# EBI-Metagenomics/deciphon

Hardware: AMD Instinct MI355X
Metric: GCUPS (Viterbi DP cell updates/sec) (higher is better)
Workload: dtype f32

## Files before the change

deciphon_amd/csrc/dcp_types.h:

```cpp
#pragma once
#include <stdint.h>

#define DCP_TABLE_SIZE 1364
#define DCP_NUM_TRANS 8
#define DCP_NUM_XTRANS 13
#define DCP_XT_STRIDE 16
#define DCP_REF_LANES 8
#define DCP_MODEL_MAX 16384

enum { DCP_BM, DCP_MM, DCP_MI, DCP_MD, DCP_IM, DCP_II, DCP_DM, DCP_DD };
enum { DCP_RR, DCP_SN, DCP_NN, DCP_SB, DCP_NB, DCP_EB, DCP_JB, DCP_EJ, DCP_JJ, DCP_EC, DCP_CC, DCP_ET, DCP_CT };

struct DcpCodeRow
{
  uint32_t c[8];
};

#define DCP_SP_STRIDE 8
#define DCP_ROW_HDR 4
#define DCP_MAX_STRIPS 8

struct DcpProfileDev
{
  int32_t K;
  int32_t Kp;
  int32_t Q;
  int32_t W;
  int64_t rows_off;
  int64_t trans_off;
  int64_t pad0, pad1;
};

struct DcpProblem
{
  int32_t profile;
  int32_t L;
  int64_t code_row;
  int32_t xt_row;
  int32_t out;
  int64_t trellis;
};

struct DcpPack
{
  int32_t profile;
  int32_t Lmax;
  int32_t L[16];
  int32_t xt_row[16];
  int32_t out[16];
  uint32_t code_row[16];
};

#ifdef __HIPCC__
#define DCP_HDI __host__ __device__ inline
// ... 25 lines not shown
```

deciphon_amd/csrc/engine.cpp:

```cpp
#include "../../include/deciphon_hip.h"
#include "dcp_db.h"
#include "dcp_errors.h"
#include "dcp_types.h"
#include "host_logic.h"
#include "viterbi_kernels.h"

#include <algorithm>
#include <atomic>
#include <deque>
#include <math.h>
#include <stdio.h>
#include <stdlib.h>
#include <string.h>
#include <string>
#include <thread>
#include <vector>

namespace
{

template <class T> struct DevBuf
{
  T *p = nullptr;
  size_t cap = 0;
// ... 90 lines not shown
    }
    auto const t0 = std::chrono::steady_clock::now();
    unsigned char *p = nullptr;
    if (hipMalloc((void **)&p, want) != hipSuccess)
    {
      (void)hipGetLastError();
      return nullptr;
    }
    double const ms = std::chrono::duration<double, std::milli>(std::chrono::steady_clock::now() - t0).count();
    alloc_ms += ms;
    if (getenv("DECIPHON_HIP_TIMING")) fprintf(stderr, "TableArena: chunk %zu, %.2f GB in %.1f ms\n", chunks.size(), (double)want / 1e9, ms);
    chunks.push_back(Chunk{p, want, bytes});
    held += want;
    placed += bytes;
    return p;
  }
};

struct HostProfile
{
  int K, Kp, Q, W, cls;
  int pack = -1;
  bool narrow = false;
  int64_t pool_off;
  std::string accession;
};

struct PathResult
{
  int K = 0, L = 0;
  float score = 0;
  size_t trellis_off = 0;
  bool has_trellis = false;
  bool trellis_on_host = false;
  uint32_t const *steps = nullptr;
  int32_t nsteps = 0;
  std::vector<uint32_t> owned;
};

}

struct dcp_hip
{
  int device = 0;
  hipStream_t stream = nullptr;
  hipStream_t qstream[DCP_NUM_CLASSES] = {nullptr};
// ... 657 lines not shown
  for (int b = 0; b < 3; ++b)
  {
    if (x->bank[b].done_ev) (void)hipEventDestroy(x->bank[b].done_ev);
    if (x->bank[b].up_ev) (void)hipEventDestroy(x->bank[b].up_ev);
  }
  for (int c = 0; c < DCP_NUM_PACK_SHAPES; ++c)
  {
    if (x->pstream[c]) (void)hipStreamDestroy(x->pstream[c]);
    if (x->pjoin_ev[c]) (void)hipEventDestroy(x->pjoin_ev[c]);
  }
  for (int c = 0; c < DCP_NUM_CLASSES; ++c)
  {
    if (x->nstream[c]) (void)hipStreamDestroy(x->nstream[c]);
    if (x->njoin_ev[c]) (void)hipEventDestroy(x->njoin_ev[c]);
  }
  if (x->fork_ev) (void)hipEventDestroy(x->fork_ev);
  if (x->stream) (void)hipStreamDestroy(x->stream);
  delete x;
}

char const *dcp_hip_strerror(struct dcp_hip const *x) { return x ? x->err.c_str() : "no engine"; }


static size_t profile_floats(int Kp)
{
  size_t const floats = (size_t)DCP_TABLE_SIZE * ((size_t)Kp + DCP_ROW_HDR) + (size_t)DCP_NUM_TRANS * (size_t)Kp;
  return (floats + 3) & ~(size_t)3;
}

static int describe(dcp_hip *x, int K, char const *accession, HostProfile &hp)
{
  if (K < 1 || K > DCP_MODEL_MAX) return fail(x, DCP_ELARGECORESIZE, "core size out of range");
  int const cls = dcp_class_of(K);
  if (cls < 0) return fail(x, DCP_ELARGECORESIZE, "core size beyond DCP_MAX_CORE_SIZE (16383: state ids keep 14 bits for k + 1)");
  hp.K = K;
  hp.cls = cls;
  dcp_class_shape(cls, &hp.Q, &hp.W);
  hp.Kp = 64 * hp.Q * hp.W;
  if (cls == DCP_STRIP_CLASS) hp.Kp *= (K + hp.Kp - 1) / hp.Kp;
  hp.pool_off = 0;
  hp.accession = accession ? accession : "";
  hp.narrow = K <= dcp_class_narrow_limit(cls);
  hp.pack = dcp_pack_shape_of(K);
  if (hp.pack >= 0)
  {
    int pq = 0, ps = 0;
    dcp_pack_shape(hp.pack, &pq, &ps);
    if (hp.W != 1 || ps * pq > hp.Kp) hp.pack = -1;
  }
  return 0;
}

static int ensure_pool(dcp_hip *x, size_t floats)
{
  if (floats <= x->d_pool.cap) return 0;
  HIP_TRY(x, hipStreamSynchronize(x->stream), DCP_EFUNCUSE);
  DevBuf<float> bigger;
  HIP_TRY(x, bigger.reserve(std::max(floats, x->d_pool.cap + x->d_pool.cap / 2)), DCP_ENOMEM);
  if (x->pool_used)
    HIP_TRY(x, hipMemcpy(bigger.p, x->d_pool.p, x->pool_used * sizeof(float), hipMemcpyDeviceToDevice), DCP_EFUNCUSE);
  x->d_pool.release();
  x->d_pool.p = bigger.p;
  x->d_pool.cap = bigger.cap;
  bigger.p = nullptr;
  bigger.cap = 0;
// ... 12 lines not shown
  x->profiles.push_back(hp);
  ++x->gen;
  return 0;
}

static bool delete_costs_ok(float const *trans, int K, int Kp)
{
  for (int k = 0; k < K; ++k)
    if (!(trans[(size_t)DCP_MD * Kp + k] >= 0.0f) || !(trans[(size_t)DCP_DD * Kp + k] >= 0.0f)) return false;
  return true;
}

int dcp_hip_add_profile(struct dcp_hip *x, int K, float const *trans, float const *match, float const *null_cost,
                        float const *bg_cost, int *index)
{
  if (!x || !trans || !match || !null_cost || !bg_cost) return DCP_EFUNCUSE;
  if (outstanding_batches(x)) return fail(x, DCP_EFUNCUSE, "cost batches are outstanding (dcp_hip_cost_hits_begin): end them first");
  HIP_TRY(x, hipSetDevice(x->device), DCP_EFUNCUSE);
  HostProfile hp;
  int rc = describe(x, K, nullptr, hp);
  if (rc) return rc;
  int const Kp = hp.Kp;
  size_t const stride = (size_t)Kp + DCP_ROW_HDR;
  std::vector<float> buf(profile_floats(Kp), INFINITY);
  float *r = buf.data();
  float *t = r + (size_t)DCP_TABLE_SIZE * stride;
  for (int id = 0; id < DCP_NUM_TRANS; ++id) memcpy(t + (size_t)id * Kp, trans + (size_t)id * K, sizeof(float) * K);
  if (!delete_costs_ok(t, K, Kp)) return fail(x, DCP_EFUNCUSE, "negative (or NaN) delete cost: costs are -log-probabilities");
  for (int c = 0; c < DCP_TABLE_SIZE; ++c)
  {
    float *hdr = r + (size_t)c * stride;
    hdr[0] = null_cost[c];
    hdr[1] = bg_cost[c];
    hdr[2] = hdr[3] = 0.0f;
    memcpy(hdr + DCP_ROW_HDR, match + (size_t)c * K, sizeof(float) * K);
  }
  return push_profile(x, hp, buf, index);
}

int dcp_hip_add_protein(struct dcp_hip *x, int K, float const *node_trans, float const *node_emission,
                        float const *BMk, float const *null_lprob, float const *bg_lprob, int *index)
{
  if (!x || !node_trans || !node_emission || !BMk || !null_lprob || !bg_lprob) return DCP_EFUNCUSE;
  if (outstanding_batches(x)) return fail(x, DCP_EFUNCUSE, "cost batches are outstanding (dcp_hip_cost_hits_begin): end them first");
  HIP_TRY(x, hipSetDevice(x->device), DCP_EFUNCUSE);
  HostProfile hp;
  int rc = describe(x, K, nullptr, hp);
  if (rc) return rc;
  std::vector<float> buf(profile_floats(hp.Kp), INFINITY);
  float *r = buf.data();
  float *t = r + (size_t)DCP_TABLE_SIZE * ((size_t)hp.Kp + DCP_ROW_HDR);
  dcp_setup_profile(K, hp.Kp, node_trans, node_emission, BMk, null_lprob, bg_lprob, t, r);
  if (!delete_costs_ok(t, K, hp.Kp)) return fail(x, DCP_EFDATA, "positive (or NaN) delete log-probability in the protein");
  return push_profile(x, hp, buf, index);
}

int dcp_hip_load_dcp(struct dcp_hip *x, char const *path, int first, int count)
{
  if (!x || !path) return DCP_EFUNCUSE;
  if (outstanding_batches(x)) return fail(x, DCP_EFUNCUSE, "cost batches are outstanding (dcp_hip_cost_hits_begin): end them first");
  HIP_TRY(x, hipSetDevice(x->device), DCP_EFUNCUSE);
  DcpDbReader db;
  int rc = db.open(path);
  if (rc) return fail(x, rc, "cannot open database");
  int const N = db.num_proteins();
  if (first < 0 || first > N) return fail(x, DCP_EINVALPART, "first protein out of range");
  int const last = count < 0 ? N : std::min(N, first + count);
  int const n = last - first;
  if (n <= 0)
  {
    ++x->gen;
    return 0;
  }

  std::vector<HostProfile> hps((size_t)n);
  std::vector<size_t> off((size_t)n + 1, 0);
  for (int i = 0; i < n; ++i)
  {
    int K = 0;
    std::string acc;
    if ((rc = db.read_protein_head(first + i, K, acc))) return fail(x, rc, "cannot read protein");
    if ((rc = describe(x, K, acc.c_str(), hps[(size_t)i]))) return rc;
    off[(size_t)i + 1] = off[(size_t)i] + profile_floats(hps[(size_t)i].Kp);
  }
  if ((rc = ensure_pool(x, x->pool_used + off[(size_t)n]))) return rc;

  size_t chunk_floats = std::max<size_t>((size_t)64 << 20, profile_floats(DCP_MAX_CORE_SIZE));
  if (char const *e = getenv("DECIPHON_HIP_STAGE_MB"))
  {
    size_t largest = 0;
    for (int i = 0; i < n; ++i) largest = std::max(largest, off[(size_t)i + 1] - off[(size_t)i]);
    chunk_floats = std::max<size_t>(((size_t)std::max(atol(e), 1L) << 20) / sizeof(float), largest);
  }
  int chunks = 0;
  float *stage[2] = {nullptr, nullptr};
  hipEvent_t done[2] = {nullptr, nullptr};
  bool busy[2] = {false, false};
  auto cleanup = [&]() {
    (void)hipStreamSynchronize(x->stream);
    for (int b = 0; b < 2; ++b)
    {
      if (stage[b]) (void)hipHostFree(stage[b]);
      if (done[b]) (void)hipEventDestroy(done[b]);
    }
  };
  for (int b = 0; b < 2; ++b)
  {
    if (hipHostMalloc((void **)&stage[b], std::min(chunk_floats, off[(size_t)n]) * sizeof(float), hipHostMallocDefault) !=
            hipSuccess ||
        hipEventCreateWithFlags(&done[b], hipEventDisableTiming) != hipSuccess)
// ... 14 lines not shown
    }
    float *buf = stage[b];
    std::atomic<int> next_protein{i0}, bad{0};
    auto work = [&]() {
      DcpProtein p;
      for (int i = next_protein.fetch_add(1); i < i1; i = next_protein.fetch_add(1))
      {
        int r = db.read_protein(first + i, p);
        if (r || p.core_size != hps[(size_t)i].K)
        {
          int expected = 0;
          bad.compare_exchange_strong(expected, r ? r : DCP_EFDATA);
          continue;
        }
        float *rows = buf + (off[(size_t)i] - off[(size_t)i0]);
        float *trans = rows + (size_t)DCP_TABLE_SIZE * ((size_t)hps[(size_t)i].Kp + DCP_ROW_HDR);
        dcp_setup_profile(p.core_size, hps[(size_t)i].Kp, p.trans.data(), p.emission.data(), p.BMk.data(),
                          p.null_emission.data(), p.bg_emission.data(), trans, rows);
        if (!delete_costs_ok(trans, p.core_size, hps[(size_t)i].Kp))
        {
          int expected = 0;
          bad.compare_exchange_strong(expected, DCP_EFDATA);
        }
      }
    };
    {
      unsigned nthreads = std::min<unsigned>({std::max(1u, std::thread::hardware_concurrency()), 16u, (unsigned)(i1 - i0)});
      std::vector<std::thread> pool;
      for (unsigned t = 1; t < nthreads; ++t) pool.emplace_back(work);
      work();
      for (std::thread &t : pool) t.join();
    }
    if (bad)
    {
      cleanup();
      return fail(x, bad, "cannot read protein");
    }
    size_t const floats = off[(size_t)i1] - off[(size_t)i0];
    if (hipMemcpyAsync(x->d_pool.p + x->pool_used + off[(size_t)i0], buf, floats * sizeof(float), hipMemcpyHostToDevice,
                       x->stream) != hipSuccess ||
        hipEventRecord(done[b], x->stream) != hipSuccess)
    {
      cleanup();
      return fail(x, DCP_EFUNCUSE, "staging copy failed");
    }
    busy[b] = true;
// ... 29 lines not shown
{
  if (!x || i < 0 || i >= (int)x->profiles.size()) return nullptr;
  return x->profiles[(size_t)i].accession.c_str();
}

int dcp_hip_commit_profiles(struct dcp_hip *x)
{
  if (!x) return DCP_EFUNCUSE;
  if (outstanding_batches(x)) return fail(x, DCP_EFUNCUSE, "cost batches are outstanding (dcp_hip_cost_hits_begin): end them first");
  HIP_TRY(x, hipSetDevice(x->device), DCP_EFUNCUSE);
  ++x->gen;
  if (x->committed == x->profiles.size()) return 0;
  HIP_TRY(x, hipStreamSynchronize(x->stream), DCP_EFUNCUSE);
  std::vector<DcpProfileDev> dev(x->profiles.size());
  for (size_t i = 0; i < dev.size(); ++i)
  {
    HostProfile const &hp = x->profiles[i];
    dev[i].K = hp.K;
    dev[i].Kp = hp.Kp;
    dev[i].Q = hp.Q;
    dev[i].W = hp.W;
    dev[i].rows_off = hp.pool_off;
    dev[i].trans_off = dev[i].rows_off + (int64_t)DCP_TABLE_SIZE * (hp.Kp + DCP_ROW_HDR);
    dev[i].pad0 = dev[i].pad1 = 0;
  }
  HIP_TRY(x, x->d_profiles.reserve(dev.size()), DCP_ENOMEM);
  HIP_TRY(x, hipMemcpyAsync(x->d_profiles.p, dev.data(), dev.size() * sizeof(DcpProfileDev), hipMemcpyHostToDevice,
                            x->stream),
          DCP_EFUNCUSE);
  HIP_TRY(x, hipStreamSynchronize(x->stream), DCP_EFUNCUSE);
  x->committed = x->profiles.size();
  return 0;
}

void dcp_hip_clear_profiles(struct dcp_hip *x)
{
  if (!x) return;
  if (outstanding_batches(x))
  {
    (void)refuse_outstanding(x);
    return;
  }
  ++x->gen;
  x->pool_used = 0;
  x->profiles.clear();
  x->committed = 0;
}
// ... 857 lines not shown
```

deciphon_amd/csrc/host_capi.cpp:

```cpp
#include "../../include/deciphon_host.h"
#include "dcp_db.h"
#include "dcp_errors.h"
#include "host_logic.h"

#include <string.h>
#include <string>
#include <vector>

struct dcp_db
{
  DcpDbReader reader;
};

extern "C" {

int dcp_db_open(char const *path, struct dcp_db **out)
{
  if (!path || !out) return DCP_EFUNCUSE;
  dcp_db *x = new dcp_db;
  int rc = x->reader.open(path);
  if (rc)
  {
    delete x;
    *out = nullptr;
// ... 55 lines not shown
int dcp_db_read_nuclt_dist(struct dcp_db const *x, int i, float *nucltp, float *codonm, int *gencode)
{
  if (!x) return DCP_EFUNCUSE;
  DcpDecoder d;
  int rc = x->reader.read_decoder(i, d);
  if (rc) return rc;
  if (nucltp) memcpy(nucltp, d.nucltp.data(), d.nucltp.size() * sizeof(float));
  if (codonm) memcpy(codonm, d.codonm.data(), d.codonm.size() * sizeof(float));
  if (gencode) *gencode = d.gencode;
  return 0;
}

int dcp_decode_quasi_codon(float epsilon, float const *nucltp4, float const *codonm125, uint8_t const *nt, int n,
                           uint8_t codon[3])
{
  if (!nucltp4 || !codonm125 || !nt || !codon) return DCP_EFUNCUSE;
  for (int i = 0; i < n && i < 5; ++i)
    if (nt[i] > 3) return DCP_ESEQABC;
  return dcp_decode_codon(epsilon, nucltp4, codonm125, nt, n, codon) ? 0 : DCP_EDECODON;
}

char dcp_gencode_amino_of(int gencode_id, uint8_t const codon[3]) { return dcp_gencode_amino(gencode_id, codon); }

int dcp_partition_bounds_of(int n, int32_t const *core_sizes, int nparts, int balanced, int32_t *first)
{
  if (n < 0 || !first || (balanced && n > 0 && !core_sizes)) return DCP_EFUNCUSE;
  if (nparts < 1) return DCP_EZEROPART;
  dcp_partition_bounds(n, core_sizes, nparts, balanced != 0, first);
  return 0;
}

int dcp_db_read_protein(struct dcp_db const *x, int i, float *node_trans, float *node_emission, float *BMk,
                        float *null_lprob, float *bg_lprob, char *accession, char *consensus)
{
  if (!x) return DCP_EFUNCUSE;
  DcpProtein p;
  int rc = x->reader.read_protein(i, p);
  if (rc) return rc;
  if (node_trans) memcpy(node_trans, p.trans.data(), p.trans.size() * sizeof(float));
  if (node_emission) memcpy(node_emission, p.emission.data(), p.emission.size() * sizeof(float));
  if (BMk) memcpy(BMk, p.BMk.data(), p.BMk.size() * sizeof(float));
  if (null_lprob) memcpy(null_lprob, p.null_emission.data(), p.null_emission.size() * sizeof(float));
  if (bg_lprob) memcpy(bg_lprob, p.bg_emission.data(), p.bg_emission.size() * sizeof(float));
  if (accession)
  {
    strncpy(accession, p.accession.c_str(), 31);
// ... 64 lines not shown
```

deciphon_amd/csrc/host_logic.cpp:

```cpp
#include "host_logic.h"
#include "../../include/deciphon_host.h"
#include "dcp_errors.h"

#include <algorithm>
#include <initializer_list>
#include <limits.h>
#include <math.h>
#include <stdio.h>
#include <string.h>
#include <utility>

void dcp_xtrans(int seq_size, bool multi_hits, bool hmmer3_compat, float xt[DCP_NUM_XTRANS])
{
  float const L = (float)seq_size;
  float q = 0.0f;
  float log_q = -INFINITY;
  if (multi_hits)
  {
    q = 0.5f;
    log_q = (float)log(0.5);
  }
  float const denom = L + 2 + q / (1 - q);
  float const two_q = 2 + q / (1 - q);
  float const Lp1 = L + 1;
// ... 31 lines not shown
  for (int k = 0; k + 1 < K; ++k)
  {
    float const *t = node_trans + 7 * (size_t)k;
    trans[DCP_MM * Kp + k + 1] = -t[0];
    trans[DCP_MI * Kp + k] = -t[1];
    trans[DCP_MD * Kp + k + 1] = -t[2];
    trans[DCP_IM * Kp + k + 1] = -t[3];
    trans[DCP_II * Kp + k] = -t[4];
    trans[DCP_DM * Kp + k + 1] = -t[5];
    trans[DCP_DD * Kp + k + 1] = -t[6];
  }
  trans[DCP_MI * Kp + K - 1] = INFINITY;
  trans[DCP_II * Kp + K - 1] = INFINITY;
  size_t const stride = (size_t)Kp + DCP_ROW_HDR;
  for (int c = 0; c < DCP_TABLE_SIZE; ++c)
  {
    float *hdr = rows + (size_t)c * stride;
    hdr[0] = -null_lprob[c];
    hdr[1] = -bg_lprob[c];
    hdr[2] = hdr[3] = 0.0f;
    float *row = hdr + DCP_ROW_HDR;
    for (int k = 0; k < K; ++k) row[k] = -node_emission[(size_t)k * DCP_TABLE_SIZE + c];
    for (int k = K; k < Kp; ++k) row[k] = INFINITY;
  }
}

int dcp_encode_sequence(char const *data, int64_t n, uint8_t *out)
{
  enum { A, C, G, T, U, NSYM };
  int64_t count[NSYM] = {0};
  for (int64_t i = 0; i < n; ++i)
  {
    switch (data[i] & ~0x20)
    {
    case 'A': count[A]++; break;
    case 'C': count[C]++; break;
    case 'G': count[G]++; break;
    case 'T': count[T]++; break;
    case 'U': count[U]++; break;
    default: break;
    }
  }
  if (count[T] > 0 && count[U] > 0) return DCP_ENUCLTSEQTU;

  auto pick = [&](std::initializer_list<int> set) {
    int best = *set.begin();
// ... 482 lines not shown
```

deciphon_amd/csrc/host_logic.h:

```cpp
#pragma once
#include "dcp_types.h"
#include <stdint.h>
#include <string>
#include <vector>

void dcp_xtrans(int seq_size, bool multi_hits, bool hmmer3_compat, float xt[DCP_NUM_XTRANS]);

void dcp_setup_profile(int K, int Kp, float const *node_trans, float const *node_emission, float const *BMk,
                       float const *null_lprob, float const *bg_lprob, float *trans, float *rows);

int dcp_encode_sequence(char const *data, int64_t n, uint8_t *out);

int dcp_unzip(int K, int L, uint32_t const *xnodes, uint16_t const *nodes, std::vector<int32_t> &state_ids,
              std::vector<int32_t> &seqsizes);

void dcp_state_name(int state_id, char name[8]);
bool dcp_state_is_mute(int state_id);

struct DcpHit
{
  int hit_start, hit_stop;
  int begin_step, end_step;
  int last_hit_pos;
};
bool dcp_find_hit(std::vector<int32_t> const &state_ids, std::vector<int32_t> const &seqsizes, DcpHit &hit);
bool dcp_find_hit_packed(uint32_t const *steps, int n, DcpHit &hit);

struct DcpWindow
{
  int core_size, seq_size;
  int start = -1, stop = 0, idx = -1, last_hit_pos = -1;
  DcpWindow(int seq_size_, int core_size_) : core_size(core_size_), seq_size(seq_size_) {}
// ... 21 lines not shown
```

deciphon_amd/csrc/lane_ops_gpu.h:

```cpp
#pragma once
#include <hip/hip_runtime.h>
#include <stdint.h>
#include <type_traits>

#include "dcp_types.h"

#define DCP_FN __device__ __forceinline__
#define DCP_WAVE 64

typedef float lf;
typedef uint32_t lu;
typedef bool lm;

DCP_FN lf lf_splat(float x) { return x; }
DCP_FN lu lu_splat(uint32_t x) { return x; }
DCP_FN lf lmin(lf a, lf b) { return __builtin_fminf(a, b); }
DCP_FN lf lmin3(lf a, lf b, lf c) { return __builtin_fminf(__builtin_fminf(a, b), c); }
DCP_FN lm llt(lf a, lf b) { return a < b; }
DCP_FN lm llt_u(lu a, lu b) { return a < b; }
DCP_FN lm leq(lf a, lf b) { return a == b; }
DCP_FN lm lequ(lu a, lu b) { return a == b; }
DCP_FN lm land(lm a, lm b) { return a && b; }
DCP_FN lm lor(lm a, lm b) { return a || b; }
DCP_FN lm lnot(lm a) { return !a; }
// ... 499 lines not shown
  dcp_u32x2 const b = __builtin_amdgcn_raw_buffer_load_b64(r.rsrc, voff + 16u, soff, 0);
  out[0] = __uint_as_float(a.x); out[1] = __uint_as_float(a.y); out[2] = __uint_as_float(a.z);
  out[3] = __uint_as_float(a.w); out[4] = __uint_as_float(b.x); out[5] = __uint_as_float(b.y);
}
template <> DCP_FN void load_row_q<8>(RowSrc const &r, lu voff, uint32_t soff, lf (&out)[8])
{
  dcp_u32x4 const a = __builtin_amdgcn_raw_buffer_load_b128(r.rsrc, voff, soff, 0);
  dcp_u32x4 const b = __builtin_amdgcn_raw_buffer_load_b128(r.rsrc, voff + 16u, soff, 0);
  out[0] = __uint_as_float(a.x); out[1] = __uint_as_float(a.y); out[2] = __uint_as_float(a.z);
  out[3] = __uint_as_float(a.w); out[4] = __uint_as_float(b.x); out[5] = __uint_as_float(b.y);
  out[6] = __uint_as_float(b.z); out[7] = __uint_as_float(b.w);
}

template <> DCP_FN void load_row_q<10>(RowSrc const &r, lu voff, uint32_t soff, lf (&out)[10])
{
  dcp_u32x4 const a = __builtin_amdgcn_raw_buffer_load_b128(r.rsrc, voff, soff, 0);
  dcp_u32x4 const b = __builtin_amdgcn_raw_buffer_load_b128(r.rsrc, voff + 16u, soff, 0);
  dcp_u32x2 const c = __builtin_amdgcn_raw_buffer_load_b64(r.rsrc, voff + 32u, soff, 0);
  out[0] = __uint_as_float(a.x); out[1] = __uint_as_float(a.y); out[2] = __uint_as_float(a.z);
  out[3] = __uint_as_float(a.w); out[4] = __uint_as_float(b.x); out[5] = __uint_as_float(b.y);
  out[6] = __uint_as_float(b.z); out[7] = __uint_as_float(b.w); out[8] = __uint_as_float(c.x);
  out[9] = __uint_as_float(c.y);
}
template <int Q> DCP_FN void store_q(float *__restrict__ row, lu lane, lf const (&v)[Q])
{
  typedef float dcp_f32x2 __attribute__((ext_vector_type(2)));
  typedef float dcp_f32x4 __attribute__((ext_vector_type(4)));
  float *p = row + (size_t)lane * Q;
  if constexpr (Q == 1)
    __builtin_nontemporal_store(v[0], p);
  else if constexpr (Q == 2)
  {
    dcp_f32x2 const t = {v[0], v[1]};
    __builtin_nontemporal_store(t, reinterpret_cast<dcp_f32x2 *>(p));
  }
  else if constexpr (Q == 4)
  {
    dcp_f32x4 const t = {v[0], v[1], v[2], v[3]};
    __builtin_nontemporal_store(t, reinterpret_cast<dcp_f32x4 *>(p));
  }
  else
  {
#pragma unroll
    for (int q = 0; q < Q; ++q) __builtin_nontemporal_store(v[q], p + q);
  }
}
// ... 230 lines not shown
```

deciphon_amd/csrc/viterbi_body.h:

```cpp
#pragma once
#include "dcp_types.h"

#ifndef DCP_FN
#error "include a lane_ops_*.h before viterbi_body.h"
#endif

#define DCP_INF (__builtin_inff())

#define DCP_SL(P, t) (((P) + 5 - (t)) % 5)

#ifndef DCP_LAZY_POSITIONS
#define DCP_LAZY_POSITIONS 6
#endif
constexpr int dcp_lazy_turns(int Q) { return Q >= DCP_LAZY_POSITIONS ? 1 : (DCP_LAZY_POSITIONS + Q - 1) / Q; }

#ifndef DCP_SHAPE_POLICY
#define DCP_SHAPE_POLICY(Q, W) ((W) == 1 ? ((Q) > 8 ? 7 : (Q) == 8 ? 2 : 0) : ((Q) >= 8 ? 6 : 0))
#endif
#ifndef DCP_COST_POLICY
#define DCP_COST_POLICY(Q, W) (DCP_SHAPE_POLICY(Q, W) | ((W) == 1 && ((Q) == 4 || (Q) == 5) ? 1 : 0))
#endif
template <int Q, int W, bool STORE = false, int POLICY = DCP_SHAPE_POLICY(Q, W)> struct CostWave
{
  static constexpr int TURNS = dcp_lazy_turns(Q);
// ... 26 lines not shown
  {
#pragma unroll
    for (int s = 0; s < 5; ++s)
    {
      load_q<Q>(from + (size_t)s * tabKp, g.lane, Mpre[s]);
      load_q<Q>(from + (size_t)(5 + s) * tabKp, g.lane, Ipre[s]);
      Spre[s] = load_lane(from + (size_t)10 * tabKp + s * 64 * W, g.lane);
    }
    X = load_lane(from + (size_t)10 * tabKp + 5 * 64 * W, g.lane);
  }
  lf BM[Q], MM[Q], MI[Q], MD[Q], IM[Q], II[Q], DM[Q], DD[Q];
  lf Mpre[5][Q], Ipre[5][Q], Spre[5];
  lf em[5][Q];
  lf sa, sb;
  lf X;
  lf NBv, EBv, JBv;
  lf shM, shI, shD;
  float nil[5], bgv[5];
  float ET, CT, RR;
  float E;
  RowSrc rows;
  lu voff;
  uint32_t stride_bytes;
  DcpCodeRow const *__restrict__ codes;

  DcpCodeRow cr;

  DCP_FN void fetch(int l_after, int L)
  {
#pragma unroll
    for (int t = 0; t < 5; ++t)
    {
      uint32_t const off = cr.c[t] * stride_bytes;
      load_row_hdr(rows, off, nil[t], bgv[t]);
      load_row_q<Q>(rows, voff, off, em[t]);
    }
    cr = codes[l_after <= L ? l_after : L];
  }

  DCP_FN void init(float const *__restrict__ pool, DcpProfileDev const &pf, DcpCodeRow const *__restrict__ code_rows,
                   float const *__restrict__ xt)
  {
#ifndef DCP_WAVE_PRIO
#define DCP_WAVE_PRIO(Q, W) ((W) > 1 || (Q) >= 6 ? 3 : (Q) >= 4 ? 2 : (Q) == 3 ? 1 : 0)
#endif
    wave_priority<DCP_WAVE_PRIO(Q, W)>();
    g.init();
    lu const lane = g.lane;
    int const Kp = pf.Kp;
    stride_bytes = (uint32_t)(Kp + DCP_ROW_HDR) * 4u;
    rows = rowsrc_make(pool + pf.rows_off, (uint32_t)DCP_TABLE_SIZE * stride_bytes);
    voff = row_lane_offset<Q>(lane);
    codes = code_rows;
    float const *__restrict__ trans = pool + pf.trans_off;
    load_q<Q>(trans + DCP_BM * Kp, lane, BM);
    load_q<Q>(trans + DCP_MM * Kp, lane, MM);
    load_q<Q>(trans + DCP_MI * Kp, lane, MI);
    load_q<Q>(trans + DCP_MD * Kp, lane, MD);
    load_q<Q>(trans + DCP_IM * Kp, lane, IM);
    load_q<Q>(trans + DCP_II * Kp, lane, II);
    load_q<Q>(trans + DCP_DM * Kp, lane, DM);
    load_q<Q>(trans + DCP_DD * Kp, lane, DD);
    NBv = lf_pin(xt[DCP_NB]);
    EBv = lf_pin(xt[DCP_EB]);
    JBv = lf_pin(xt[DCP_JB]);
    shM = shI = shD = lf_splat(DCP_INF);
    g.put_tdd(DD);
    if constexpr (STASH)
    {
      g.template stash_q<Q, SLOTS>(0, MD);
      g.template stash_q<Q, SLOTS>(1, DD);
      g.template stash_q<Q, SLOTS>(2, II);
      g.template stash_q<Q, SLOTS>(3, MI);
      if constexpr (STASH6)
// ... 886 lines not shown
```

deciphon_amd/csrc/viterbi_kernels.h:

```cpp
#pragma once
#include "dcp_types.h"
#include <hip/hip_runtime.h>

#define DCP_NUM_CLASSES 12
#define DCP_STRIP_CLASS 11
#define DCP_STRIP_POSITIONS 2048
#define DCP_MAX_CORE_SIZE 16383
#define DCP_RING_FLOATS ((size_t)10 * DCP_MAX_STRIPS * DCP_STRIP_POSITIONS)
#define DCP_RING_SLOTS 1024
int dcp_class_of(int K);
void dcp_class_shape(int cls, int *Q, int *W);

#define DCP_NUM_PACK_SHAPES 11
int dcp_pack_shape_of(int K);
void dcp_pack_shape(int shape, int *Q, int *S);

struct DcpLaunch
{
  float const *pool;
  DcpProfileDev const *profiles;
  DcpProblem const *problems;
  DcpCodeRow const *code_rows;
  float const *xt_table;
  float *out;
  unsigned char *arena;
  float *ring = nullptr;
  int nprob;
  hipStream_t stream;
};

hipError_t dcp_launch_cost(int cls, DcpLaunch const &a);
int dcp_class_narrow_limit(int cls);
hipError_t dcp_launch_cost_narrow(int cls, DcpLaunch const &a);
hipError_t dcp_launch_path(int cls, DcpLaunch const &a);
hipError_t dcp_launch_unzip(DcpLaunch const &a, uint32_t *steps, int64_t const *step_off, int32_t *nsteps);
hipError_t dcp_launch_cost_ckpt(int cls, DcpLaunch const &a, int64_t const *ckpt_addr, int B);
hipError_t dcp_launch_cost_store(int cls, DcpLaunch const &a, int64_t const *ckpt_addr, int B, int block, int G = 0, int it = 0);
hipError_t dcp_launch_traceback(DcpLaunch const &a, uint32_t *steps, int64_t const *step_off, int32_t *nsteps,
                                DcpTraceState *states, int B, int block, int G = 0, int it = 0);
hipError_t dcp_launch_path_blocks(int cls, DcpLaunch const &a, int64_t const *ckpt_addr, int B, uint32_t *steps,
                                  int64_t const *step_off, int32_t *nsteps, DcpTraceState *states);
hipError_t dcp_launch_replay(DcpLaunch const &a, int64_t const *table_addr, int64_t const *scratch_addr, int max_rows);
hipError_t dcp_launch_compact_steps(uint32_t const *steps, int64_t const *step_off, int64_t const *compact_off,
                                    uint32_t *out, int n, hipStream_t stream);
hipError_t dcp_launch_cost_pack(int shape, DcpLaunch const &a, DcpPack const *packs, int npack, uint32_t ncode_rows);
hipError_t dcp_launch_lrt_filter(float const *out, int n, uint32_t *hits, hipStream_t stream);
int dcp_pack_lds_waves(int shape);
hipError_t dcp_launch_cost_pack_lds(int shape, DcpLaunch const &a, DcpPack const *packs, int2 const *groups, int ngroups,
                                    uint32_t ncode_rows);
hipError_t dcp_launch_cost_fused(DcpLaunch const &a);
hipError_t dcp_launch_encode(unsigned char const *nt, int64_t const *seq_off, int64_t const *row_off, int nseq,
                             int64_t max_len, DcpCodeRow *rows, hipStream_t stream);
```

deciphon_amd/csrc/viterbi_kernels.hip:

```cpp
#include <stdlib.h>

#include "lane_ops_gpu.h"
#include "viterbi_body.h"
#include "viterbi_pack.h"
#include "traceback.h"
#include "viterbi_kernels.h"
#include "row_replay.h"

template <class T> __device__ __forceinline__ T *dcp_global(uintptr_t address)
{
  return (T *)(__attribute__((address_space(1))) T *)address;
}

__device__ __forceinline__ int dcp_xcd_remap_any(int b, int n)
{
  int const q = n >> 3, r = n & 7, x = b & 7;
  return (x < r ? x * (q + 1) : r * (q + 1) + (x - r) * q) + (b >> 3);
}
__device__ __forceinline__ int dcp_xcd_remap(int b, int n)
{
  return n < 16384 ? b : dcp_xcd_remap_any(b, n);
}

#ifndef DCP_COST_WAVES
// ... 760 lines not shown

hipError_t dcp_launch_cost(int cls, DcpLaunch const &a)
{
  if (a.nprob <= 0) return hipSuccess;
  switch (cls)
  {
  case 0: return launch_cost_qw<1, 1>(a);
  case 1: return launch_cost_qw<2, 1>(a);
  case 2: return launch_cost_qw<3, 1>(a);
  case 3: return launch_cost_qw<4, 1>(a);
  case 4: return launch_cost_qw<6, 1>(a);
  case 5: return launch_cost_qw<8, 1>(a);
  case 6: return launch_cost_qw<6, 2>(a);
  case 7: return launch_cost_qw<4, 4>(a);
  case 8: return launch_cost_qw<6, 4>(a);
  case 9: return launch_cost_qw<8, 4>(a);
  case 10: return launch_cost_qw<8, 8>(a);
  case DCP_STRIP_CLASS: return launch_strip<false>(a);
  default: return hipErrorInvalidValue;
  }
}

int dcp_class_narrow_limit(int cls) { return cls == 4 ? 320 : cls == 5 ? 448 : cls == 6 ? 640 : 0; }

hipError_t dcp_launch_cost_narrow(int cls, DcpLaunch const &a)
{
  if (a.nprob <= 0) return hipSuccess;
  switch (cls)
  {
  case 4: return launch_cost_qw<5, 1>(a);
  case 5: return launch_cost_qw<7, 1>(a);
  case 6: return launch_cost_qw<10, 1>(a);
  default: return hipErrorInvalidValue;
  }
}

template <int Q, int W>
static hipError_t launch_store_qw(DcpLaunch const &a, int64_t const *ckpt_addr, int B, int block, int G, int it)
{
  hipLaunchKernelGGL((dcp_cost_store_kernel<Q, W>), dim3((unsigned)a.nprob * (unsigned)(G > 0 ? G : 1)), dim3(64 * W), 0,
                     a.stream, a.pool, a.profiles, a.problems, a.code_rows, a.xt_table, a.arena, ckpt_addr, B, block, G, it,
                     a.out, a.nprob);
  return hipGetLastError();
}

hipError_t dcp_launch_cost_store(int cls, DcpLaunch const &a, int64_t const *ckpt_addr, int B, int block, int G, int it)
{
  if (a.nprob <= 0) return hipSuccess;
  switch (cls)
  {
  case 0: return launch_store_qw<1, 1>(a, ckpt_addr, B, block, G, it);
  case 1: return launch_store_qw<2, 1>(a, ckpt_addr, B, block, G, it);
  case 2: return launch_store_qw<3, 1>(a, ckpt_addr, B, block, G, it);
  case 3: return launch_store_qw<4, 1>(a, ckpt_addr, B, block, G, it);
  case 4: return launch_store_qw<6, 1>(a, ckpt_addr, B, block, G, it);
// ... 195 lines not shown
```

deciphon_amd/host.py:

```python
from __future__ import annotations

import ctypes as C
import os

import numpy as np

from .hip import HipError, load_library

TABLE_SIZE = 1364


class _Window(C.Structure):
    _fields_ = [(n, C.c_int32) for n in ("core_size", "seq_size", "start", "stop", "idx", "last_hit_pos")]


def _lib():
    L = load_library()
    if getattr(L, "_host_ready", False):
        return L
    vp, i32 = C.c_void_p, C.c_int
    L.dcp_db_open.argtypes = [C.c_char_p, C.POINTER(vp)]
    L.dcp_db_close.argtypes = [vp]
    L.dcp_db_close.restype = None
    L.dcp_db_num_proteins.argtypes = [vp]
    L.dcp_db_epsilon.argtypes = [vp]
    L.dcp_db_epsilon.restype = C.c_float
    L.dcp_db_entry_dist.argtypes = [vp]
    L.dcp_db_has_ga.argtypes = [vp]
    L.dcp_db_protein_offset.argtypes = [vp, i32]
    L.dcp_db_protein_offset.restype = C.c_int64
    L.dcp_db_protein_core_size.argtypes = [vp, i32, C.POINTER(i32)]
    L.dcp_db_read_protein.argtypes = [vp, i32, vp, vp, vp, vp, vp, C.c_char_p, C.c_char_p]
    L.dcp_db_read_nuclt_dist.argtypes = [vp, i32, vp, vp, C.POINTER(i32)]
    L.dcp_decode_quasi_codon.argtypes = [C.c_float, vp, vp, vp, i32, vp]
    L.dcp_gencode_amino_of.argtypes = [i32, vp]
    L.dcp_gencode_amino_of.restype = C.c_char
    L.dcp_db_core_sizes.argtypes = [vp, vp]
    L.dcp_db_partition_bounds.argtypes = [vp, i32, i32, vp]
    L.dcp_partition_bounds_of.argtypes = [i32, vp, i32, i32, vp]
    L.dcp_partition_size.argtypes = [C.c_long, C.c_long, C.c_long]
    L.dcp_partition_size.restype = C.c_long
    L.dcp_window_count.argtypes = [C.c_int64, i32]
    L.dcp_window_count.restype = C.c_int64
    L.dcp_scan_plan_chunks.argtypes = [i32, vp, i32, vp, C.c_double, C.c_double, C.c_int64, C.c_int64, i32, vp, vp,
                                       C.POINTER(i32)]
    L.dcp_window_setup.argtypes = [C.POINTER(_Window), i32, i32]
    L.dcp_window_setup.restype = None
    L.dcp_window_next.argtypes = [C.POINTER(_Window)]
    L.dcp_trellis_unzip.argtypes = [i32, i32, vp, vp, i32, vp, vp, C.POINTER(i32)]
    L.dcp_path_hit.argtypes = [i32, vp, vp, vp]
    L.dcp_state_name_of.argtypes = [i32, C.c_char_p]
    L.dcp_state_name_of.restype = None
    L.dcp_state_is_mute_id.argtypes = [i32]
    L.dcp_lrt_of.argtypes = [C.c_float, C.c_float]
    L.dcp_lrt_of.restype = C.c_float
    L.dcp_hmm_open.argtypes = [C.c_char_p, i32, C.POINTER(vp)]
    L.dcp_hmm_close.argtypes = [vp]
    L.dcp_hmm_close.restype = None
    L.dcp_hmm_count.argtypes = [vp]
    L.dcp_hmm_count.restype = C.c_long
    L.dcp_hmm_next.argtypes = [vp]
    L.dcp_hmm_end.argtypes = [vp]
    L.dcp_hmm_core_size.argtypes = [vp]
    L.dcp_hmm_has_ga.argtypes = [vp]
    L.dcp_hmm_read.argtypes = [vp, vp, vp, vp, vp, C.c_char_p, C.c_char_p]
    L._host_ready = True
# ... 145 lines not shown
    return int(_lib().dcp_partition_size(nelems, nparts, idx))


class WindowIter:

    def __init__(self, seq_size: int, core_size: int):
        self.lib = _lib()
        self.w = _Window()
        self.lib.dcp_window_setup(C.byref(self.w), seq_size, core_size)

    def next(self):
        if not self.lib.dcp_window_next(C.byref(self.w)):
            return None
        return self.w.idx, self.w.start, self.w.stop

    def set_last_hit_position(self, pos: int) -> None:
        self.w.last_hit_pos = pos


def window_count(seq_size: int, core_size: int) -> int:
    return int(_lib().dcp_window_count(int(seq_size), int(core_size)))


def plan_chunks(core_sizes, read_lengths, first_cells: float, later_cells: float, max_pairs: int, max_windows: int):
    L = _lib()
    K = np.ascontiguousarray(core_sizes, np.int32)
    R = np.ascontiguousarray(read_lengths, np.int32)
    cap = 64
    while True:
        chunks = np.zeros((cap, 4), np.int32)
        windows = np.zeros(cap, np.int64)
        n = C.c_int(0)
        rc = L.dcp_scan_plan_chunks(len(K), K.ctypes.data_as(C.c_void_p), len(R), R.ctypes.data_as(C.c_void_p),
                                    float(first_cells), float(later_cells), int(max_pairs), int(max_windows), cap,
                                    chunks.ctypes.data_as(C.c_void_p), windows.ctypes.data_as(C.c_void_p), C.byref(n))
        if rc == 20 and n.value > cap:
            cap = n.value
            continue
        if rc:
            raise HipError(rc)
        return chunks[: n.value].copy(), windows[: n.value].copy()


def unzip(K: int, L: int, xnodes: np.ndarray, nodes: np.ndarray):
    lib = _lib()
    xnodes = np.ascontiguousarray(xnodes, np.uint32)
# ... 56 lines not shown
```

include/deciphon_host.h:

```cpp
#ifndef DECIPHON_HOST_H
#define DECIPHON_HOST_H

#include <stdint.h>

#ifdef __cplusplus
extern "C" {
#endif

struct dcp_db;
int dcp_db_open(char const *path, struct dcp_db **out);
void dcp_db_close(struct dcp_db *);
int dcp_db_num_proteins(struct dcp_db const *);
float dcp_db_epsilon(struct dcp_db const *);
int dcp_db_entry_dist(struct dcp_db const *);
int dcp_db_has_ga(struct dcp_db const *);
int64_t dcp_db_protein_offset(struct dcp_db const *, int i);
int dcp_db_protein_core_size(struct dcp_db const *, int i, int *core_size);
int dcp_db_read_protein(struct dcp_db const *, int i, float *node_trans, float *node_emission, float *BMk,
                        float *null_lprob, float *bg_lprob, char *accession, char *consensus);

int dcp_db_read_nuclt_dist(struct dcp_db const *, int i, float *nucltp, float *codonm, int *gencode);
int dcp_decode_quasi_codon(float epsilon, float const *nucltp4, float const *codonm125, uint8_t const *nt, int n,
                           uint8_t codon[3]);
char dcp_gencode_amino_of(int gencode_id, uint8_t const codon[3]);

struct dcp_hmm;
int dcp_hmm_open(char const *path, int gencode_id, struct dcp_hmm **out);
void dcp_hmm_close(struct dcp_hmm *);
long dcp_hmm_count(struct dcp_hmm const *);
int dcp_hmm_next(struct dcp_hmm *);
int dcp_hmm_end(struct dcp_hmm const *);
int dcp_hmm_core_size(struct dcp_hmm const *);
int dcp_hmm_has_ga(struct dcp_hmm const *);
int dcp_hmm_read(struct dcp_hmm const *, float *trans, float *BMk, float *nucltp, float *codonm, char *accession,
                 char *consensus);

long dcp_partition_size(long nelems, long nparts, long idx);
int dcp_db_core_sizes(struct dcp_db const *, int32_t *core_sizes);
int dcp_db_partition_bounds(struct dcp_db const *, int nparts, int balanced, int32_t *first);
int dcp_partition_bounds_of(int n, int32_t const *core_sizes, int nparts, int balanced, int32_t *first);

int64_t dcp_window_count(int64_t seq_size, int core_size);
int dcp_scan_plan_chunks(int nprof, int32_t const *core_sizes, int nreads, int32_t const *read_lengths,
                         double first_cells, double later_cells, int64_t max_pairs, int64_t max_windows, int cap,
                         int32_t *chunks, int64_t *windows, int *nchunks);
#define DCP_SCAN_FIRST_CHUNK_CELLS 1.0e10
#define DCP_SCAN_CHUNK_PAIRS (1 << 21)
#define DCP_SCAN_CHUNK_WINDOWS (4 << 20)

struct dcp_window
{
  int32_t core_size, seq_size;
  int32_t start, stop, idx, last_hit_pos;
};
void dcp_window_setup(struct dcp_window *, int seq_size, int core_size);
int dcp_window_next(struct dcp_window *);

int dcp_trellis_unzip(int K, int L, uint32_t const *xnodes, uint16_t const *nodes, int cap, int32_t *state_ids,
                      int32_t *seqsizes, int *nsteps);

int dcp_path_hit(int nsteps, int32_t const *state_ids, int32_t const *seqsizes, int32_t hit[5]);

void dcp_state_name_of(int state_id, char *name);
int dcp_state_is_mute_id(int state_id);

// ... 8 lines not shown
```

Measured before the change: 831.2.

## Add chunk-interleaved copy of emission cost rows for coalesced narrow-kernel loads

For narrow profiles with Q of 5 or 10, the host now builds a second copy of each emission cost row with columns permuted so that each lane's Q values are grouped into contiguous 4-wide chunks laid out lane-interleaved across the wavefront. The cost kernel detects this copy through new profile fields and loads emissions with b128/b96/b64 buffer loads at the new offsets, aiming for better coalescing of the per-step row reads. In exchange, profile memory grows by roughly one extra table per narrow profile and host staging does more work; Q=7 profiles do not get the copy.

```diff
diff --git a/deciphon_amd/csrc/dcp_types.h b/deciphon_amd/csrc/dcp_types.h
--- a/deciphon_amd/csrc/dcp_types.h
+++ b/deciphon_amd/csrc/dcp_types.h
@@ -28,8 +28,11 @@
   int32_t W;
   int64_t rows_off;
   int64_t trans_off;
-  int64_t pad0, pad1;
+  int64_t cost_rows_off;
+  int64_t cost_shape;
 };
+#define DCP_COST_SHAPE(Q, W) ((Q) * 256 + (W))
+#define DCP_COST_ORDER_HDR 32
 
 struct DcpProblem
 {
diff --git a/deciphon_amd/csrc/engine.cpp b/deciphon_amd/csrc/engine.cpp
--- a/deciphon_amd/csrc/engine.cpp
+++ b/deciphon_amd/csrc/engine.cpp
@@ -136,6 +136,7 @@
   int K, Kp, Q, W, cls;
   int pack = -1;
   bool narrow = false;
+  int cQ = 0, cW = 0;
   int64_t pool_off;
   std::string accession;
 };
@@ -839,10 +840,39 @@
 char const *dcp_hip_strerror(struct dcp_hip const *x) { return x ? x->err.c_str() : "no engine"; }
 
 
-static size_t profile_floats(int Kp)
+static size_t canonical_floats(int Kp)
 {
   size_t const floats = (size_t)DCP_TABLE_SIZE * ((size_t)Kp + DCP_ROW_HDR) + (size_t)DCP_NUM_TRANS * (size_t)Kp;
-  return (floats + 3) & ~(size_t)3;
+  return (floats + 31) & ~(size_t)31;
+}
+
+static size_t profile_floats(HostProfile const &hp)
+{
+  size_t const copy = hp.cQ ? (size_t)DCP_TABLE_SIZE * (size_t)dcp_cost_order_stride(hp.cQ, hp.cW) : 0;
+  return canonical_floats(hp.Kp) + copy;
+}
+
+static bool cost_order_pays(int Q, int W) { return W == 1 && (Q == 5 || Q == 10); }
+
+static void cost_order_shape(HostProfile &hp)
+{
+  hp.cQ = hp.cW = 0;
+  char const *e = getenv("DECIPHON_HIP_COST_ORDER");
+  if (!hp.narrow || (e && e[0] == '0')) return;
+  int const q = dcp_class_narrow_q(hp.cls);
+  if (!cost_order_pays(q, 1)) return;
+  hp.cQ = q;
+  hp.cW = 1;
+}
+
+static void stage_cost_order(HostProfile const &hp, float *staged)
+{
+  if (!hp.cQ) return;
+  dcp_cost_order_rows(hp.cQ, hp.cW, hp.K, hp.Kp, staged, staged + canonical_floats(hp.Kp));
+  char const *e = getenv("DECIPHON_HIP_COST_ORDER");
+  if (e && strcmp(e, "poison") == 0)
+    for (int c = 0; c < DCP_TABLE_SIZE; ++c)
+      memset(staged + (size_t)c * ((size_t)hp.Kp + DCP_ROW_HDR) + DCP_ROW_HDR, 0, sizeof(float) * (size_t)hp.K);
 }
 
 static int describe(dcp_hip *x, int K, char const *accession, HostProfile &hp)
@@ -858,6 +888,7 @@
   hp.pool_off = 0;
   hp.accession = accession ? accession : "";
   hp.narrow = K <= dcp_class_narrow_limit(cls);
+  cost_order_shape(hp);
   hp.pack = dcp_pack_shape_of(K);
   if (hp.pack >= 0)
   {
@@ -916,7 +947,7 @@
   if (rc) return rc;
   int const Kp = hp.Kp;
   size_t const stride = (size_t)Kp + DCP_ROW_HDR;
-  std::vector<float> buf(profile_floats(Kp), INFINITY);
+  std::vector<float> buf(profile_floats(hp), INFINITY);
   float *r = buf.data();
   float *t = r + (size_t)DCP_TABLE_SIZE * stride;
   for (int id = 0; id < DCP_NUM_TRANS; ++id) memcpy(t + (size_t)id * Kp, trans + (size_t)id * K, sizeof(float) * K);
@@ -929,6 +960,7 @@
     hdr[2] = hdr[3] = 0.0f;
     memcpy(hdr + DCP_ROW_HDR, match + (size_t)c * K, sizeof(float) * K);
   }
+  stage_cost_order(hp, r);
   return push_profile(x, hp, buf, index);
 }
 
@@ -941,11 +973,12 @@
   HostProfile hp;
   int rc = describe(x, K, nullptr, hp);
   if (rc) return rc;
-  std::vector<float> buf(profile_floats(hp.Kp), INFINITY);
+  std::vector<float> buf(profile_floats(hp), INFINITY);
   float *r = buf.data();
   float *t = r + (size_t)DCP_TABLE_SIZE * ((size_t)hp.Kp + DCP_ROW_HDR);
   dcp_setup_profile(K, hp.Kp, node_trans, node_emission, BMk, null_lprob, bg_lprob, t, r);
   if (!delete_costs_ok(t, K, hp.Kp)) return fail(x, DCP_EFDATA, "positive (or NaN) delete log-probability in the protein");
+  stage_cost_order(hp, r);
   return push_profile(x, hp, buf, index);
 }
 
@@ -975,11 +1008,11 @@
     std::string acc;
     if ((rc = db.read_protein_head(first + i, K, acc))) return fail(x, rc, "cannot read protein");
     if ((rc = describe(x, K, acc.c_str(), hps[(size_t)i]))) return rc;
-    off[(size_t)i + 1] = off[(size_t)i] + profile_floats(hps[(size_t)i].Kp);
+    off[(size_t)i + 1] = off[(size_t)i] + profile_floats(hps[(size_t)i]);
   }
   if ((rc = ensure_pool(x, x->pool_used + off[(size_t)n]))) return rc;
 
-  size_t chunk_floats = std::max<size_t>((size_t)64 << 20, profile_floats(DCP_MAX_CORE_SIZE));
+  size_t chunk_floats = std::max<size_t>((size_t)64 << 20, canonical_floats(DCP_MAX_CORE_SIZE));
   if (char const *e = getenv("DECIPHON_HIP_STAGE_MB"))
   {
     size_t largest = 0;
@@ -1040,6 +1073,7 @@
           int expected = 0;
           bad.compare_exchange_strong(expected, DCP_EFDATA);
         }
+        stage_cost_order(hps[(size_t)i], rows);
       }
     };
     {
@@ -1115,7 +1149,8 @@
     dev[i].W = hp.W;
     dev[i].rows_off = hp.pool_off;
     dev[i].trans_off = dev[i].rows_off + (int64_t)DCP_TABLE_SIZE * (hp.Kp + DCP_ROW_HDR);
-    dev[i].pad0 = dev[i].pad1 = 0;
+    dev[i].cost_rows_off = hp.cQ ? hp.pool_off + (int64_t)canonical_floats(hp.Kp) : 0;
+    dev[i].cost_shape = hp.cQ ? DCP_COST_SHAPE(hp.cQ, hp.cW) : 0;
   }
   HIP_TRY(x, x->d_profiles.reserve(dev.size()), DCP_ENOMEM);
   HIP_TRY(x, hipMemcpyAsync(x->d_profiles.p, dev.data(), dev.size() * sizeof(DcpProfileDev), hipMemcpyHostToDevice,
diff --git a/deciphon_amd/csrc/host_capi.cpp b/deciphon_amd/csrc/host_capi.cpp
--- a/deciphon_amd/csrc/host_capi.cpp
+++ b/deciphon_amd/csrc/host_capi.cpp
@@ -101,6 +101,13 @@
 
 char dcp_gencode_amino_of(int gencode_id, uint8_t const codon[3]) { return dcp_gencode_amino(gencode_id, codon); }
 
+int dcp_cost_order_map(int Q, int W, int32_t *cols)
+{
+  if (Q < 1 || W < 1 || Q * W > 64 || !cols) return 0;
+  for (int k = 0; k < 64 * Q * W; ++k) cols[k] = dcp_cost_order_col(Q, W, k);
+  return dcp_cost_order_stride(Q, W);
+}
+
 int dcp_partition_bounds_of(int n, int32_t const *core_sizes, int nparts, int balanced, int32_t *first)
 {
   if (n < 0 || !first || (balanced && n > 0 && !core_sizes)) return DCP_EFUNCUSE;
diff --git a/deciphon_amd/csrc/host_logic.cpp b/deciphon_amd/csrc/host_logic.cpp
--- a/deciphon_amd/csrc/host_logic.cpp
+++ b/deciphon_amd/csrc/host_logic.cpp
@@ -77,6 +77,32 @@
     float *row = hdr + DCP_ROW_HDR;
     for (int k = 0; k < K; ++k) row[k] = -node_emission[(size_t)k * DCP_TABLE_SIZE + c];
     for (int k = K; k < Kp; ++k) row[k] = INFINITY;
+  }
+}
+
+int dcp_cost_order_col(int Q, int W, int k)
+{
+  (void)W;
+  int const g = k / Q, q = k % Q, w = g / 64, e = g % 64, c = q / 4;
+  int const wc = Q - 4 * c < 4 ? Q - 4 * c : 4;
+  return 64 * Q * w + 256 * c + e * wc + (q - 4 * c);
+}
+
+int dcp_cost_order_stride(int Q, int W) { return DCP_COST_ORDER_HDR + 64 * Q * W; }
+
+void dcp_cost_order_rows(int Q, int W, int K, int Kp, float const *rows, float *copy)
+{
+  int const Kc = 64 * Q * W, stride = dcp_cost_order_stride(Q, W);
+  std::vector<int> col((size_t)Kc);
+  for (int k = 0; k < Kc; ++k) col[(size_t)k] = dcp_cost_order_col(Q, W, k);
+  for (int c = 0; c < DCP_TABLE_SIZE; ++c)
+  {
+    float const *hdr = rows + (size_t)c * ((size_t)Kp + DCP_ROW_HDR);
+    float const *row = hdr + DCP_ROW_HDR;
+    float *out = copy + (size_t)c * stride;
+    for (int j = 0; j < DCP_ROW_HDR; ++j) out[j] = hdr[j];
+    for (int j = DCP_ROW_HDR; j < DCP_COST_ORDER_HDR; ++j) out[j] = INFINITY;
+    for (int k = 0; k < Kc; ++k) out[DCP_COST_ORDER_HDR + col[(size_t)k]] = k < K ? row[k] : INFINITY;
   }
 }
 
diff --git a/deciphon_amd/csrc/host_logic.h b/deciphon_amd/csrc/host_logic.h
--- a/deciphon_amd/csrc/host_logic.h
+++ b/deciphon_amd/csrc/host_logic.h
@@ -8,6 +8,10 @@
 
 void dcp_setup_profile(int K, int Kp, float const *node_trans, float const *node_emission, float const *BMk,
                        float const *null_lprob, float const *bg_lprob, float *trans, float *rows);
+
+int dcp_cost_order_col(int Q, int W, int k);
+int dcp_cost_order_stride(int Q, int W);
+void dcp_cost_order_rows(int Q, int W, int K, int Kp, float const *rows, float *copy);
 
 int dcp_encode_sequence(char const *data, int64_t n, uint8_t *out);
 
diff --git a/deciphon_amd/csrc/lane_ops_gpu.h b/deciphon_amd/csrc/lane_ops_gpu.h
--- a/deciphon_amd/csrc/lane_ops_gpu.h
+++ b/deciphon_amd/csrc/lane_ops_gpu.h
@@ -545,6 +545,49 @@
   out[6] = __uint_as_float(b.z); out[7] = __uint_as_float(b.w); out[8] = __uint_as_float(c.x);
   out[9] = __uint_as_float(c.y);
 }
+
+#define DCP_COST_ORDER 1
+template <int Q> struct DcpRowChunks
+{
+  static constexpr int N = (Q + 3) / 4;
+  static constexpr int width(int c) { return Q - 4 * c < 4 ? Q - 4 * c : 4; }
+};
+
+template <int Q, int W> DCP_FN void row_chunk_offsets(lu lane, bool ordered, lu (&v)[DcpRowChunks<Q>::N])
+{
+  lu const w = lane >> 6, e = lane & 63u;
+#pragma unroll
+  for (int c = 0; c < DcpRowChunks<Q>::N; ++c)
+    v[c] = ordered ? (uint32_t)(4 * DCP_COST_ORDER_HDR) + w * (uint32_t)(256 * Q) + (uint32_t)(1024 * c) +
+                         e * (uint32_t)(4 * DcpRowChunks<Q>::width(c))
+                   : row_lane_offset<Q>(lane) + (uint32_t)(16 * c);
+}
+
+template <int Q, int C = 0>
+DCP_FN void load_row_chunks(RowSrc const &r, lu const (&v)[DcpRowChunks<Q>::N], uint32_t soff, lf (&out)[Q])
+{
+  constexpr int WC = DcpRowChunks<Q>::width(C), q0 = 4 * C;
+  if constexpr (WC == 4)
+  {
+    dcp_u32x4 const a = __builtin_amdgcn_raw_buffer_load_b128(r.rsrc, v[C], soff, 0);
+    out[q0] = __uint_as_float(a.x); out[q0 + 1] = __uint_as_float(a.y);
+    out[q0 + 2] = __uint_as_float(a.z); out[q0 + 3] = __uint_as_float(a.w);
+  }
+  else if constexpr (WC == 3)
+  {
+    dcp_u32x3 const a = __builtin_amdgcn_raw_buffer_load_b96(r.rsrc, v[C], soff, 0);
+    out[q0] = __uint_as_float(a.x); out[q0 + 1] = __uint_as_float(a.y); out[q0 + 2] = __uint_as_float(a.z);
+  }
+  else if constexpr (WC == 2)
+  {
+    dcp_u32x2 const a = __builtin_amdgcn_raw_buffer_load_b64(r.rsrc, v[C], soff, 0);
+    out[q0] = __uint_as_float(a.x); out[q0 + 1] = __uint_as_float(a.y);
+  }
+  else
+    out[q0] = __uint_as_float(__builtin_amdgcn_raw_buffer_load_b32(r.rsrc, v[C], soff, 0));
+  if constexpr (C + 1 < DcpRowChunks<Q>::N) load_row_chunks<Q, C + 1>(r, v, soff, out);
+}
+
 template <int Q> DCP_FN void store_q(float *__restrict__ row, lu lane, lf const (&v)[Q])
 {
   typedef float dcp_f32x2 __attribute__((ext_vector_type(2)));
diff --git a/deciphon_amd/csrc/viterbi_body.h b/deciphon_amd/csrc/viterbi_body.h
--- a/deciphon_amd/csrc/viterbi_body.h
+++ b/deciphon_amd/csrc/viterbi_body.h
@@ -72,6 +72,10 @@
   RowSrc rows;
   lu voff;
   uint32_t stride_bytes;
+#ifdef DCP_COST_ORDER
+  static constexpr bool ORDERED = !STORE && Q >= 5;
+  lu voffc[ORDERED ? DcpRowChunks<Q>::N : 1];
+#endif
   DcpCodeRow const *__restrict__ codes;
 
   DcpCodeRow cr;
@@ -82,6 +86,14 @@
     for (int t = 0; t < 5; ++t)
     {
       uint32_t const off = cr.c[t] * stride_bytes;
+#ifdef DCP_COST_ORDER
+      if constexpr (ORDERED)
+      {
+        load_row_hdr(rows, off, nil[t], bgv[t]);
+        load_row_chunks<Q>(rows, voffc, off, em[t]);
+        continue;
+      }
+#endif
       load_row_hdr(rows, off, nil[t], bgv[t]);
       load_row_q<Q>(rows, voff, off, em[t]);
     }
@@ -99,7 +111,20 @@
     lu const lane = g.lane;
     int const Kp = pf.Kp;
     stride_bytes = (uint32_t)(Kp + DCP_ROW_HDR) * 4u;
-    rows = rowsrc_make(pool + pf.rows_off, (uint32_t)DCP_TABLE_SIZE * stride_bytes);
+    int64_t rows_off = pf.rows_off;
+#ifdef DCP_COST_ORDER
+    if constexpr (ORDERED)
+    {
+      bool const copy = pf.cost_rows_off != 0 && pf.cost_shape == DCP_COST_SHAPE(Q, W);
+      if (copy)
+      {
+        rows_off = pf.cost_rows_off;
+        stride_bytes = 4u * (uint32_t)(DCP_COST_ORDER_HDR + 64 * Q * W);
+      }
+      row_chunk_offsets<Q, W>(lane, copy, voffc);
+    }
+#endif
+    rows = rowsrc_make(pool + rows_off, (uint32_t)DCP_TABLE_SIZE * stride_bytes);
     voff = row_lane_offset<Q>(lane);
     codes = code_rows;
     float const *__restrict__ trans = pool + pf.trans_off;
diff --git a/deciphon_amd/csrc/viterbi_kernels.h b/deciphon_amd/csrc/viterbi_kernels.h
--- a/deciphon_amd/csrc/viterbi_kernels.h
+++ b/deciphon_amd/csrc/viterbi_kernels.h
@@ -31,6 +31,7 @@
 
 hipError_t dcp_launch_cost(int cls, DcpLaunch const &a);
 int dcp_class_narrow_limit(int cls);
+int dcp_class_narrow_q(int cls);
 hipError_t dcp_launch_cost_narrow(int cls, DcpLaunch const &a);
 hipError_t dcp_launch_path(int cls, DcpLaunch const &a);
 hipError_t dcp_launch_unzip(DcpLaunch const &a, uint32_t *steps, int64_t const *step_off, int32_t *nsteps);
diff --git a/deciphon_amd/csrc/viterbi_kernels.hip b/deciphon_amd/csrc/viterbi_kernels.hip
--- a/deciphon_amd/csrc/viterbi_kernels.hip
+++ b/deciphon_amd/csrc/viterbi_kernels.hip
@@ -806,15 +806,16 @@
 }
 
 int dcp_class_narrow_limit(int cls) { return cls == 4 ? 320 : cls == 5 ? 448 : cls == 6 ? 640 : 0; }
+int dcp_class_narrow_q(int cls) { return cls == 4 ? 5 : cls == 5 ? 7 : cls == 6 ? 10 : 0; }
 
 hipError_t dcp_launch_cost_narrow(int cls, DcpLaunch const &a)
 {
   if (a.nprob <= 0) return hipSuccess;
-  switch (cls)
-  {
-  case 4: return launch_cost_qw<5, 1>(a);
-  case 5: return launch_cost_qw<7, 1>(a);
-  case 6: return launch_cost_qw<10, 1>(a);
+  switch (dcp_class_narrow_q(cls))
+  {
+  case 5: return launch_cost_qw<5, 1>(a);
+  case 7: return launch_cost_qw<7, 1>(a);
+  case 10: return launch_cost_qw<10, 1>(a);
   default: return hipErrorInvalidValue;
   }
 }
diff --git a/deciphon_amd/host.py b/deciphon_amd/host.py
--- a/deciphon_amd/host.py
+++ b/deciphon_amd/host.py
@@ -42,6 +42,7 @@
     L.dcp_partition_size.restype = C.c_long
     L.dcp_window_count.argtypes = [C.c_int64, i32]
     L.dcp_window_count.restype = C.c_int64
+    L.dcp_cost_order_map.argtypes = [i32, i32, vp]
     L.dcp_scan_plan_chunks.argtypes = [i32, vp, i32, vp, C.c_double, C.c_double, C.c_int64, C.c_int64, i32, vp, vp,
                                        C.POINTER(i32)]
     L.dcp_window_setup.argtypes = [C.POINTER(_Window), i32, i32]
@@ -233,6 +234,14 @@
     return int(_lib().dcp_window_count(int(seq_size), int(core_size)))
 
 
+def cost_order_map(Q: int, W: int):
+    cols = np.zeros(64 * Q * W, np.int32)
+    stride = int(_lib().dcp_cost_order_map(int(Q), int(W), cols.ctypes.data_as(C.c_void_p)))
+    if stride <= 0:
+        raise ValueError(f"no cost-order map for Q={Q}, W={W}")
+    return cols, stride
+
+
 def plan_chunks(core_sizes, read_lengths, first_cells: float, later_cells: float, max_pairs: int, max_windows: int):
     L = _lib()
     K = np.ascontiguousarray(core_sizes, np.int32)
diff --git a/include/deciphon_host.h b/include/deciphon_host.h
--- a/include/deciphon_host.h
+++ b/include/deciphon_host.h
@@ -41,6 +41,7 @@
 int dcp_partition_bounds_of(int n, int32_t const *core_sizes, int nparts, int balanced, int32_t *first);
 
 int64_t dcp_window_count(int64_t seq_size, int core_size);
+int dcp_cost_order_map(int Q, int W, int32_t *cols);
 int dcp_scan_plan_chunks(int nprof, int32_t const *core_sizes, int nreads, int32_t const *read_lengths,
                          double first_cells, double later_cells, int64_t max_pairs, int64_t max_windows, int cap,
                          int32_t *chunks, int64_t *windows, int *nchunks);
```

Measured after the change: 846.4, median of 6. 1.8% higher.
